# mryndzionek/composable-sdr

Measured on AMD Instinct MI355X. Metric: MS/s CF32 throughput, 256-ch PFB+FM pipeline, higher is better.
Workload: dtype f32; 1 GPU; cfg3: 256-ch firpfbch(m=7,As=80)+dcBlocker+freqdem(kf=0.3) on synthetic CF32, AGC off (-a 0), 262144 frames/step (512 MiB in, 256 MiB out), HBM-resident; channels=256, demod=fm, mix=False, route=fused-256|k_tile256<FM>, preheat_steps=11199, collective=none, rccl_ranks=1

## Files before the change

composable_sdr_amd/csrc/capi.hip:

```cpp
#include "../../include/csdr.h"
#include "csdr_internal.h"
#include "fused.h"

#include <cmath>
#include <cstdio>
#include <cstring>
#include <new>

namespace csdr {
const char *last_error();
}
using namespace csdr;

namespace {

struct DevGuard {
    int prev = -1; bool ok = true;
    DevGuard() = default;
    explicit DevGuard(int dev) { select(dev); }
    void select(int dev) {
        if (hipGetDevice(&prev) != hipSuccess) { ok = false; return; }
        if (dev >= 0 && dev != prev && hipSetDevice(dev) != hipSuccess) ok = false;
    }
    ~DevGuard() { if (prev >= 0) (void)hipSetDevice(prev); }
// ... 766 lines not shown
int csdr_symsync_get_taps(const csdr_symsync *h, float *mf, float *dmf)
{
    if (!h) return CSDR_ERR_INVALID;
    if (mf) std::memcpy(mf, h->d.mf.data(), sizeof(float) * h->d.mf.size());
    if (dmf) std::memcpy(dmf, h->d.dmf.data(), sizeof(float) * h->d.dmf.size());
    return CSDR_OK;
}

}

namespace {
constexpr uint32_t ST1 = 1u << 1, ST2 = 1u << 2, ST4 = 1u << 4, ST8 = 1u << 8, ST_ANY = ~0u;
struct RouteRow {
    uint32_t M;
    uint32_t strides;
    bool (*supported)(uint32_t M, uint32_t p);
    int (*create)(const FusedConfig &cfg, ChainPlan **out);
    const char *path_prefix;
    double dc_window;
    const char *name, *run_sized, *other, *agc_tail;
};
const RouteRow ROUTES[] = {
    {256, ST1 | ST2 | ST4 | ST8, plan256_supported, plan256_create, "fused-256|", 6 * 4096.0, "fused-256",
     "k_run256v2<FM | CF32[, G]> (whole band: calls of >= 1024 whole tiles of 16 frames; interleaved shards G = 2, 4, 8: every whole tile)",
     "k_tile256<FM | CF32> (look-back tile kernel: chunk-sized calls, ragged ends, and contiguous channel shards at every size) [+ k_shard_gather]",
     "channelizer -> CF32 plane (tile-major for run-sized calls of whole tiles) -> k_agc_spec_tm | k_agc_spec -> k_agc_fix [-> k_mix]"},
    {64, ST1, plan64_supported, plan64_create, "fused-", 6 * 4096.0, "fused-k_run64",
     "k_run64v2 (CF32 output, whole band, nf % 64 == 0, >= 8 tiles of 64 frames per run)", "k_run64<FM | CF32> (FM output, shards, ragged calls)",
     "k_run64v2 -> CF32 plane (tile-major, run-sized calls) -> k_agc_spec_tm | k_run64<CF32> -> k_agc_spec; -> k_agc_fix [-> k_mix]"},
    {1024, ST1 | ST2 | ST4 | ST8, plan1024_supported, plan1024_create, "fused-", 6 * 4096.0, "fused-k_run1024",
     "k_run1024v3<FM | CF32> (whole band, calls of whole 4-frame tiles; a call that ends inside a 128-byte line stores the front part of it); "
     "k_shard1024<FM | CF32, G> (interleaved shards G = 4, 8: fold of the aliasing branches behind the FIR + a (1024 / G)-point DFT across the lanes; run-sized calls of whole tiles); "
     "k_run1024v2<FM, 2> (interleaved shards G = 2, FM output)",
     "k_run1024<FM | CF32> (ragged calls, contiguous shards, the other calls of interleaved shards) [+ k_pfb1024_fixup, k_shard_gather1024]", "k_run1024v3<CF32> -> CF32 plane (tile-major) -> k_agc_spec_tm | k_run1024<CF32> -> k_agc_spec; -> k_agc_fix [-> k_mix]"},
    {4096, ST1, plan4096_supported, plan4096_create, "fused-4096|", 7 * 4096.0, "fused-4096",
     "k_front4096 (DC blocker + pre-mix + FIR, branch-tiled: four sibling workgroups per frame, radix-4 split of the DFT on the registers) -> z (8 B / sample) "
     "-> k_back4096<CF32 | FM | FM,mix> (four 1024-point DFTs per frame, 16-frame blocks, whole 128-byte lines per row) [-> k_mix4096_finish]; whole band; "
     "DeNo --mix without the AGC keeps the any-M route's mix identity",
     "the same kernels (any call size; short calls use fewer runs)", "k_front4096 -> k_back4096<CF32> -> CF32 plane (tile-major: calls of whole 16-frame blocks, >= 4096 frames) -> k_agc_spec_tm | k_agc_spec -> k_agc_fix [-> k_mix]"},
    {0, ST_ANY, nullptr, nullptr, nullptr, 0.0, "generic",
     "k_dc_tile -> k_pfb_fir (M = 1024, forced generic: k_pfb1024) -> k_fft_r16 | k_fft_pow2 | k_dft_direct [interleaved shard: k_fold + (M / G)-point DFT] "
     "-> k_transpose_fm | k_mix_frames | k_transpose;  DeNo --mix over all channels: k_dc_fold + k_mixid_finish (M % 4096 == 0) | k_dc_tile + k_branch0_fir "
     "(the sum of all bins of a frame is M x branch 0);  DeNo --mix of an interleaved shard (M % 4096 == 0, G = 2, 4, 8): k_dc_fold8 + k_mixid_shard_finish "
     "(the shard's channel sum is M / G x the phasor sum of the G surviving branches)",
     "the same kernels (any call size)", "... -> k_transpose -> k_agc_spec -> k_agc_fix [-> k_fm] [-> k_mix]"},
};
const RouteRow *route_select(uint32_t M, uint32_t p, uint32_t G, uint32_t flags, const DcParams *dc)
// ... 853 lines not shown
```

composable_sdr_amd/csrc/fused_common.h:

```cpp
#pragma once
#include "fused.h"

#include <cmath>
#include <cstdlib>
#include <vector>

namespace csdr {
namespace {

constexpr int M256 = 256;
constexpr int P = 14;
constexpr int NB = 16;
constexpr int FS_X = 272;
constexpr int FS_Z = 289;
constexpr int RS_Z = 18;
constexpr int RS_Y = 17;
constexpr int LDS_F2 = 16 * FS_Z;
constexpr int E_OFF = 4096;
constexpr int LOOKBACK = 10;
constexpr unsigned SPIN_LIMIT = 1u << 24;

typedef unsigned long long u64;
typedef float v2f __attribute__((ext_vector_type(2)));

// ... 330 lines not shown
__host__ __device__ __forceinline__ void run_range(const RunSplit &sp, uint32_t w, uint32_t &first, uint32_t &last)
{
    const uint32_t s = w / sp.rps, i = w - s * sp.rps;
    first = sp.base[s] + (uint32_t)((unsigned long long)i * sp.tiles[s] / sp.rps);
    last = sp.base[s] + (uint32_t)((unsigned long long)(i + 1) * sp.tiles[s] / sp.rps);
}

struct RunArgs {
    TileArgs t;
    RunSplit split;
    PhaseK pk;
    uint32_t nruns;
    float l2beta;
    uint32_t prio_div;
    uint32_t trace_light;
    const float4 *prev_tail;
    uint32_t indep;
    uint32_t pair_align;
    uint32_t wu_batch6;
    uint32_t wu, wu_rot;
    uint32_t tile_step;
    uint32_t nowu;
    float2 *cpre, *side;
};
constexpr int DCFIX_F = 113;

__device__ __forceinline__ float2 wg_sum(float2 v, float2 *red, int tid)
{
#pragma unroll
    for (int d = 32; d >= 1; d >>= 1) { v.x += __shfl_xor(v.x, d); v.y += __shfl_xor(v.y, d); }
    if ((tid & 63) == 0) red[tid >> 6] = v;
    __syncthreads();
    const float2 r = cadd(cadd(red[0], red[1]), cadd(red[2], red[3]));
    __syncthreads();
    return r;
}

__device__ __forceinline__ void row_scan4(float &x0, float &x1, float &x2, float &x3, float &s0, float &s1, float &s2, float &s3,
                                          float b1, float b2, float b4, float b8, float na)
{
    asm volatile(
        "v_mov_b32_e32 %4, %0\n\t"
        "v_mov_b32_e32 %5, %1\n\t"
        "v_mov_b32_e32 %6, %2\n\t"
        "v_mov_b32_e32 %7, %3\n\t"
        "v_fmac_f32_dpp %4, %4, %8 row_shr:1 row_mask:0xf bank_mask:0xf\n\t"
// ... 74 lines not shown
```

composable_sdr_amd/csrc/fused_v2_common.h:

```cpp
#pragma once
#include "fused_common.h"

namespace csdr {
namespace {

typedef float v4f __attribute__((ext_vector_type(4)));
#ifndef V2_DMA_AUX
#define V2_DMA_AUX ""
#endif
#ifndef V2_DMA_AUX_STREAM
#define V2_DMA_AUX_STREAM V2_DMA_AUX
#endif

__device__ __forceinline__ void bar()
{
    asm volatile("s_waitcnt lgkmcnt(0)\n\ts_barrier" ::: "memory");
}
__device__ __forceinline__ float opaque_v(float x) { asm volatile("" : "+v"(x)); return x; }

__device__ __forceinline__ unsigned dma_offset(int tid)
{
    const int wave = tid >> 6, lane = tid & 63;
    const int slot = 64 * wave + lane, q = slot >> 3, i = (slot & 7) ^ ((q >> 1) & 7);
    return (unsigned)(8 * q + i) * 16u;
// ... 90 lines not shown
    const v2f aA = mnA * rcA, aB = mnB * rcB;
    const v2f zA = aA * aA, zB = aB * aB;
    const v2f refv = {k.ref, k.ref};
    const v2f sA = aA * refv, sB = aB * refv;
    v2f pA = __builtin_elementwise_fma((v2f){k.c[7], k.c[7]}, zA, (v2f){k.c[6], k.c[6]});
    v2f pB = __builtin_elementwise_fma((v2f){k.c[7], k.c[7]}, zB, (v2f){k.c[6], k.c[6]});
#pragma unroll
    for (int i = 5; i >= 0; i--) {
        pA = __builtin_elementwise_fma(pA, zA, (v2f){k.c[i], k.c[i]});
        pB = __builtin_elementwise_fma(pB, zB, (v2f){k.c[i], k.c[i]});
    }
    const v2f tA = pA * sA, tB = pB * sB;
    const v2f hpv = {k.hp, k.hp}, piv = {k.pi, k.pi};
    const v2f thA = hpv - tA, thB = hpv - tB;
    const v2f uA = {sel_abs_gt(q[0].y, q[0].x, thA.x, tA.x), sel_abs_gt(q[1].y, q[1].x, thA.y, tA.y)};
    const v2f uB = {sel_abs_gt(q[2].y, q[2].x, thB.x, tB.x), sel_abs_gt(q[3].y, q[3].x, thB.y, tB.y)};
    const v2f wA = piv - uA, wB = piv - uB;
    m[0] = copysignf(sel_neg(q[0].x, wA.x, uA.x), q[0].y);
    m[1] = copysignf(sel_neg(q[1].x, wA.y, uA.y), q[1].y);
    m[2] = copysignf(sel_neg(q[2].x, wB.x, uB.x), q[2].y);
    m[3] = copysignf(sel_neg(q[3].x, wB.y, uB.y), q[3].y);
}

template <int CTRL> __device__ __forceinline__ float dpp_keep(float old, float v)
{
    return __int_as_float(__builtin_amdgcn_update_dpp(__float_as_int(old), __float_as_int(v), CTRL, 0xf, 0xf, false));
}

}
template <size_t OFF> __device__ __forceinline__ unsigned kernarg_u32_s()
{
    unsigned v = 0;
#if defined(__HIP_DEVICE_COMPILE__)
    typedef __attribute__((address_space(4))) const char *kptr;
    kptr ka = (kptr)__builtin_amdgcn_kernarg_segment_ptr();
    asm volatile("s_load_dword %0, %1, %2\n\ts_waitcnt lgkmcnt(0)" : "=s"(v) : "s"(ka), "n"(OFF) : "memory");
#endif
    return v;
}
template <size_t OFF> __device__ __forceinline__ float2 *kernarg_ptr_s()
{
    float2 *p = nullptr;
#if defined(__HIP_DEVICE_COMPILE__)
    typedef __attribute__((address_space(4))) const char *kptr;
    kptr ka = (kptr)__builtin_amdgcn_kernarg_segment_ptr();
    unsigned long long v;
// ... 8 lines not shown
```

composable_sdr_amd/csrc/kernels_fused.hip:

```cpp
#include "fused_common.h"
#include <cstring>

namespace csdr {

namespace {

#define STAMP(i) do { if (A.trace && tid == 0) A.trace[(size_t)b * 16 + (i)] = __builtin_amdgcn_s_memtime(); } while (0)

template <bool FM>
__global__ __launch_bounds__(256) void k_tile256(TileArgs A)
{
    __shared__ __attribute__((aligned(16))) float2 R[LDS_F2];
    __shared__ float2 tw_s[M256];
    __shared__ float2 Tt[2][16];
    __shared__ float2 carry_s[2];
    __shared__ unsigned tile_s;

    const int tid = threadIdx.x;
    if (tid == 0) tile_s = atomicAdd(A.ticket, 1u);
    tw_s[tid] = A.tw[tid];
    __syncthreads();
    const unsigned b = tile_s;
    if (b >= A.nb) return;
    STAMP(0);
// ... 267 lines not shown
{
    const unsigned i = blockIdx.x * 256u + threadIdx.x;
    dst[i] = src[i];
}

__global__ __launch_bounds__(64) void k_shard_gather(const float *__restrict__ src, float *__restrict__ dst, uint32_t c0, uint32_t G, uint32_t rem,
                                                     uint32_t nf, uint32_t t0, uint32_t w)
{
    const uint32_t m = blockIdx.x;
    for (uint32_t i = threadIdx.x; i < rem * w; i += 64) dst[((size_t)m * nf + t0) * w + i] = src[(size_t)(c0 + G * m) * rem * w + i];
}

struct FusedPlan : ChainPlan {
    using ChainPlan::ChainPlan;
    std::string kernel;
    uint32_t max_nb = 0, epoch = 0;
    float *d_taps = nullptr;
    float2 *d_tw = nullptr, *d_wpre = nullptr;
    float2 *d_yhist[2] = {nullptr, nullptr}, *d_vend[2] = {nullptr, nullptr}, *d_rp[2] = {nullptr, nullptr};
    unsigned *d_ticket = nullptr, *d_yflag = nullptr, *d_status = nullptr;
    u64 *d_agg = nullptr, *d_ylast = nullptr;
    float2 *d_cpre = nullptr, *d_side = nullptr, *d_rt = nullptr;
    bool nowu = false;
    u64 *d_trace = nullptr;
    uint32_t run_min_tiles = 1024;
    float slot_weight[8] = {1.f, 1.f, 1.f, 1.f, 1.f, 1.f, 1.f, 1.f};
    uint32_t resident_wgs_v2 = 512;
    bool use_v3 = false;
    float *d_shard_tail = nullptr;
    float4 *d_tail[3] = {nullptr, nullptr, nullptr};
    int tail_w = 0;
    bool tail_valid = false, save_tails = false;
    TileArgs proto;

    int init();
    const char *name() const override { return kernel.c_str(); }
    bool tile_major_ok(uint32_t nf) const override;
    void keep_tail() override { save_tails = cfg.G == 1; }
    bool can_overlap(uint32_t nf) const override;
    bool tail_recorded() const override { return save_tails && tail_valid; }
    int status(unsigned *st) override;
    int trace(unsigned long long *out, uint32_t ntiles) override;
    int reset_state(hipStream_t s) override;
    int run(const FusedCall &call, void *out, hipStream_t s, KernelTimer *timer) override;
    bool v2_call(uint32_t nf) const { return cfg.G == 1 && cfg.c0 == 0 && cfg.C == cfg.M && nf / NB >= run_min_tiles; }
};
// ... 79 lines not shown
    for (int i = 0; i < 3; i++) {
        if ((r = mem.alloc(&d_tail[i], sizeof(float4) * 2048 * (WU + 1)))) return r;
        CSDR_HIP(hipMemset(d_tail[i], 0, sizeof(float4) * 2048 * (WU + 1)));
    }
    tail_valid = true;
    if ((r = mem.alloc(&d_ticket, sizeof(unsigned)))) return r;
    if ((r = mem.alloc(&d_status, sizeof(unsigned)))) return r;
    if ((r = mem.alloc(&d_yflag, sizeof(unsigned) * max_nb))) return r;
    if ((r = mem.alloc(&d_agg, sizeof(u64) * 2 * max_nb))) return r;
    if ((r = mem.alloc(&d_ylast, sizeof(u64) * (size_t)cfg.M * max_nb))) return r;
    if (const char *e = diag_env("CSDR_RUN_MIN_TILES")) run_min_tiles = (uint32_t)atol(e);
    if (cfg.mix && (r = mem.alloc(&d_premix, (size_t)cfg.C * cfg.max_nf * (cfg.fm ? 4 : 8)))) return r;
    if (diag_env("CSDR_TRACE")) {
        if ((r = mem.alloc(&d_trace, sizeof(u64) * 16 * max_nb))) return r;
        CSDR_HIP(hipMemset(d_trace, 0, sizeof(u64) * 16 * max_nb));
    }
    nowu = cfg.G == 1 && cfg.c0 == 0 && cfg.C == cfg.M && cfg.dc_block && dc_window_ok(cfg.dc, (DCFIX_F - 1) * 256.0) &&
           !(diag_env("CSDR_NOWU") && atoi(diag_env("CSDR_NOWU")) == 0);
    if (nowu) {
        if ((r = mem.alloc(&d_cpre, sizeof(float2) * 2050))) return r;
        if ((r = mem.alloc(&d_side, sizeof(float2) * 2048 * 4 * DCFIX_F))) return r;
        if ((r = mem.alloc(&d_rt, sizeof(float2) * 2 * DCFIX_F * 4))) return r;
        CSDR_HIP(hipMemset(d_cpre, 0, sizeof(float2) * 2050));
    }
    CSDR_HIP(hipMemcpy(d_taps, cfg.taps, sizeof(float) * cfg.M * cfg.p, hipMemcpyHostToDevice));
    std::vector<float2> tw(cfg.M);
    for (uint32_t k1 = 0; k1 < 16; k1++)
        for (uint32_t b1 = 0; b1 < 16; b1++) {
            const double a = -2.0 * 3.14159265358979323846 * (double)(b1 * k1) / (double)cfg.M;
            tw[16 * k1 + b1] = make_float2((float)std::cos(a), (float)std::sin(a));
        }
    const std::vector<float2> wpre = premix_table();
    CSDR_HIP(hipMemcpy(d_tw, tw.data(), sizeof(float2) * cfg.M, hipMemcpyHostToDevice));
    CSDR_HIP(hipMemcpy(d_wpre, wpre.data(), sizeof(float2) * 2 * cfg.M, hipMemcpyHostToDevice));
    if (nowu) {
        std::vector<float2> rt((size_t)2 * DCFIX_F * 4);
        dc_state_response(cfg, wpre.data(), 15u, (uint32_t)DCFIX_F, 126u, rt.data());
        CSDR_HIP(hipMemcpy(d_rt, rt.data(), sizeof(float2) * rt.size(), hipMemcpyHostToDevice));
    }
    CSDR_HIP(hipMemset(d_status, 0, sizeof(unsigned)));
    CSDR_HIP(hipMemset(d_yflag, 0, sizeof(unsigned) * max_nb));
    CSDR_HIP(hipMemset(d_agg, 0, sizeof(u64) * 2 * max_nb));

    TileArgs &A = proto;
    A = TileArgs{};
    A.taps = d_taps; A.tw = d_tw; A.wpre = d_wpre;
// ... 71 lines not shown
        RA.t = A; RA.pk = phase_consts(c.fm_ref);
        uint32_t nruns = v3 ? cus : resident_wgs_v2;
        if (v3) { if (const char *e = diag_env("CSDR_V3_RUNS")) nruns = (uint32_t)atol(e); }
        if (nruns > A.nb / 8) nruns = A.nb / 8;
        if (nruns < 1) nruns = 1;
        RA.nruns = nruns;
        static const float v2_weight_cf[8] = {1.2f, 0.8f, 1.f, 1.f, 1.f, 1.f, 1.f, 1.f};
        static const float v2_weight_fm[8] = {1.24f, 0.76f, 1.f, 1.f, 1.f, 1.f, 1.f, 1.f};
        const float *v2_weight = c.fm ? v2_weight_fm : v2_weight_cf;
        static const float equal_weight[8] = {1.f, 1.f, 1.f, 1.f, 1.f, 1.f, 1.f, 1.f};
        static const bool pd_equal = diag_env("CSDR_PD_EQUAL") != nullptr;
        RA.split = make_split(A.nb, nruns, cus, (call.indep && pd_equal) ? equal_weight : ((v2 && !diag_env("CSDR_RUN_WEIGHTS")) ? v2_weight : slot_weight));
        { const char *e = diag_env("CSDR_PRIO_ROT"); RA.prio_div = e ? (atoi(e) ? cus : 0u) : (v2 ? 0u : cus); }
        { const char *e = diag_env("CSDR_TRACE"); RA.trace_light = (e && atoi(e) == 2) ? 1u : 0u; }
        { const char *e = diag_env("CSDR_WU"); RA.wu = e ? (uint32_t)atoi(e) : (uint32_t)WU; }
        { const char *e = diag_env("CSDR_WU_ROT"); RA.wu_rot = e ? (uint32_t)atoi(e) : 0u; }
        RA.pair_align = (v2 && (c.fm || diag_env("CSDR_PAIR_ALIGN_CF"))) ? 1u : 0u;
        { const char *e = diag_env("CSDR_WU_BATCH6"); RA.wu_batch6 = e ? (uint32_t)atoi(e) : 1u; }
        RA.l2beta = c.dc_block ? (float)std::log2((double)c.dc.beta) : -1000.0f;
        RA.tile_step = call.tile_major ? c.C * 128u : (uint32_t)NB * (c.fm ? 4u : 8u);
        const bool whole = nf == nb_full * NB;
        RA.indep = call.indep ? 1u : 0u;
        RA.nowu = (nowu && !shard && !v3 && !RA.indep && nruns >= 2 && nruns <= 2048) ? 1u : 0u;
        RA.cpre = d_cpre; RA.side = d_side;
        RA.prev_tail = d_tail[tail_w];
        if (save_tails && !shard && v2 && whole && nb_full >= WU + 1) {
            const int nxt = (tail_w + 1) % 3;
            static const bool nocopy = diag_env("CSDR_PD_NOCOPY") != nullptr;
            if (!nocopy) hipLaunchKernelGGL(k_save_tail, dim3(2048 * (WU + 1) / 256), dim3(256), 0, s,
                                            reinterpret_cast<const float4 *>(call.d_in + (size_t)(nb_full - (WU + 1)) * 4096), d_tail[nxt]);
            if (call.ev_tail) CSDR_HIP(hipEventRecord(call.ev_tail, s));
            tail_w = nxt; tail_valid = true;
        } else tail_valid = false;
        if (timer && (r = timer->begin(s))) return r;
        if (nb_full == 0) {  }
#ifdef CSDR_WITH_RUN256_V3
        else if (v3) { if ((r = run256_v3_launch(&RA, c.fm, nruns, s))) return r; }
#endif
        else if ((r = run256_v2_launch(&RA, c.fm, c.G, nruns, s))) return r;
        if (RA.nowu && nb_full && (r = run256_dcfix_launch(&RA, c.fm, nruns, d_rt, s))) return r;
        if (timer && (r = timer->end(s))) return r;
        const uint32_t rem = nf - nb_full * NB;
        if (rem) {
            if (nb_full) cur ^= 1;
            TileArgs T = proto;
            T.x = call.d_in + (size_t)nb_full * NB * c.M; T.out = A.out;
            if (shard) { T.c0 = 0; T.C = c.M; T.out = d_shard_tail; }
            T.yhist_in = d_yhist[cur]; T.yhist_out = d_yhist[cur ^ 1];
            T.vend_in = d_vend[cur];   T.vend_out = d_vend[cur ^ 1];
            T.rp_in = d_rp[cur];       T.rp_out = d_rp[cur ^ 1];
            if (++epoch == 0) epoch = 1;
            T.epoch = epoch; T.nf = rem; T.nb = 1; T.out_stride = nf; T.out_t0 = nb_full * NB;
            if (shard) { T.out_stride = rem; T.out_t0 = 0; }
            T.parity0 = (uint32_t)((frames_done + nb_full * NB) & 1);
            CSDR_HIP(hipMemsetAsync(d_ticket, 0, sizeof(unsigned), s));
            if (c.fm) hipLaunchKernelGGL(k_tile256<true>, dim3(1), dim3(256), 0, s, T);
            else hipLaunchKernelGGL(k_tile256<false>, dim3(1), dim3(256), 0, s, T);
            if (shard) hipLaunchKernelGGL(k_shard_gather, dim3(c.C), dim3(64), 0, s, (const float *)d_shard_tail, (float *)A.out, c.c0, c.G, rem,
                                          nf, nb_full * NB, c.fm ? 1u : 2u);
        }
    } else {
        kernel = c.fm ? "k_tile256<FM>" : "k_tile256<CF32>";
        tail_valid = false;
// ... 30 lines not shown
```

composable_sdr_amd/csrc/kernels_fused_v2.hip:

```cpp
#ifndef V2_FM_PACKED
#define V2_FM_PACKED 1
#endif
#ifndef V2_ABLATE
#define V2_ABLATE 0
#endif

#ifndef V2_COLSCAN
#define V2_COLSCAN 0
#endif
#ifndef V2_PAIR
#define V2_PAIR 1
#endif
#ifndef V2_STORE_AUX
#define V2_STORE_AUX ""
#endif
#ifndef V2_PAIR_CF
#define V2_PAIR_CF 0
#endif
#ifndef V2_BAR_E
#define V2_BAR_E 0
#endif
#ifndef V2_PAD
#define V2_PAD 1
#endif
// ... 3 lines not shown

#include "fused_v2_common.h"
#include <cstddef>
#include <type_traits>

namespace csdr {
namespace {

constexpr unsigned V2_FSB = 2048u + (V2_PAD ? 128u : 0u);
constexpr int V2_FS2 = (int)V2_FSB / 8;
constexpr int V2_BUF = 16 * V2_FS2;
constexpr int V2_STASH = 2 * V2_BUF;
constexpr int V2_F2 = V2_STASH + 256 + 32 + 256 + (V2_COLSCAN ? 512 : 0);
#define V2_ZSW(f) (V2_PAD ? (((f) >> 1) & 7) : ((f) & 7))
#ifndef V2_RSWN
#define V2_RSWN V2_PAD
#endif
#define V2_RSW(a) (V2_RSWN ? ((a) & 7) : (((a) >> 1) & 7))

struct V2Args {
    RunArgs r;
};

template <bool FM, int G>
__global__ __launch_bounds__(256, 2) void k_run256v2(V2Args VA)
{
    static_assert(G == 1 || G == 2 || G == 4 || G == 8, "interleaved shards: G = 2, 4, 8");
    constexpr int NK1 = 16 / G;
    const RunArgs &RA = VA.r;
    const TileArgs &A = RA.t;
    __shared__ __attribute__((aligned(16))) float2 L[V2_F2];
    float2 *R = L, *ST = L + V2_STASH, *Tt = ST + 256, *red = Tt + 16;
    float2 *tw_s = red + 16;
    float2 *TRc = tw_s + 256, *Ec = TRc + 256;
    (void)TRc; (void)Ec;
    float2 *H = L + V2_BUF;
    float2 *E = ST;
    const int tid = threadIdx.x, j = tid;
    const unsigned w = blockIdx.x;
    unsigned first, last;
    run_range(RA.split, w, first, last);
    if (RA.pair_align) {
        first &= ~1u;
        if (last != A.nb) last &= ~1u;
    }
    const float4 *x4 = reinterpret_cast<const float4 *>(A.x);
    const int col_off = 16 * (j >> 4) + 2 * (((j & 15) >> 1) ^ V2_RSW(j >> 4)) + (j & 1);
    const unsigned goff = V2_RSWN ? dma_offset_rsw(tid) : dma_offset(tid);
    const unsigned wave_u = (unsigned)__builtin_amdgcn_readfirstlane(tid >> 6);
    const unsigned lds_wave = (unsigned)(size_t)(__attribute__((address_space(3))) float2 *)R + V2_FSB * (wave_u >> 1) + 1024u * (wave_u & 1u);

#ifndef V2_TRACE
#define V2_TRACE 0
#endif
// ... 1 lines not shown
#define V2LSTAMP(i) do { if (A.trace && RA.trace_light && tid == 0) A.trace[(size_t)first * 16 + (i)] = __builtin_amdgcn_s_memrealtime(); } while (0)
#else
#define V2LSTAMP(i) do { } while (0)
#endif
    V2LSTAMP(0);
    const bool cold = w > 0 || RA.indep;
    const int halo = (int)first - 1;
    auto tile_ptr = [&](int t) -> const float4 * { return t >= 0 ? x4 + (size_t)t * 2048 : RA.prev_tail + (size_t)(WU + 1 + t) * 2048; };
    if (first < last) dma_tile<false, 2 * V2_FSB>(x4 + (size_t)first * 2048, goff, lds_wave);
    if (cold) dma_tile<false, 2 * V2_FSB>(tile_ptr(halo), goff, lds_wave + (unsigned)(V2_BUF * 8));
    float h[P];
#pragma unroll
    for (int n = 0; n < P; n++) h[n] = A.taps[(M256 - 1 - j) + n * M256];
    float2 Wa = A.wpre[(A.parity0 & 1) * M256 + j], Wb = A.wpre[((A.parity0 & 1) ^ 1) * M256 + j];
    if (G > 1) {
        const int n = ((j >> 4) * (int)A.c0) & 15;
        const float C1 = 0.92387953251128674f, S1 = 0.38268343236508977f, R2 = 0.70710678118654752f;
        const int m4 = n & 3, qd = n >> 2;
        const float2 e = m4 == 0 ? make_float2(1.f, 0.f) : (m4 == 1 ? make_float2(C1, -S1) : (m4 == 2 ? make_float2(R2, -R2) : make_float2(S1, -C1)));
        const float2 rot = qd == 0 ? e : (qd == 1 ? make_float2(e.y, -e.x) : (qd == 2 ? make_float2(-e.x, -e.y) : make_float2(-e.y, e.x)));
        Wa = cmul(Wa, rot); Wb = cmul(Wb, rot);
    }
    tw_s[tid] = A.tw[tid];
    float2 wa[NB], wb[NB];
#pragma unroll
    for (int f = 0; f < NB; f++) { wa[f] = make_float2(0.f, 0.f); wb[f] = make_float2(0.f, 0.f); }
    float2 c;
    float2 w2 = make_float2(0.f, 0.f);

    if (!cold) {
        c = A.vend_in[0];
#pragma unroll
        for (int f = 3; f < NB; f++) wa[f] = A.yhist_in[(f - 3) * M256 + j];
    } else {
        const int h0 = RA.nowu ? halo : (RA.indep ? halo - (int)RA.wu : (halo > (int)RA.wu ? halo - (int)RA.wu : 0));
        const unsigned nwu = (unsigned)(halo - h0);
        float4 raw[8];
        float wt0, wt1;
        {
            const int wave = tid >> 6, lane = tid & 63;
            const int slot = 64 * wave + lane, q = slot >> 3;
            const int i = (slot & 7) ^ ((q >> 1) & 7);
            const int n = 16 * q + 2 * i;
            wt0 = exp2f((float)(4095 - n) * RA.l2beta);
            wt1 = exp2f((float)(4094 - n) * RA.l2beta);
        }
// ... 72 lines not shown
            const float2 s2 = (n == P - 1) ? w2 : wa[NB - 1 - n];
            acc = __builtin_elementwise_fma((v2f){s2.x, s2.y}, (v2f){h[n], h[n]}, acc);
        }
        H[j] = to_f2(acc);
        __syncthreads();
        v2f vv[16];
        if (tid < 16) {
#pragma unroll
            for (int a = 0; a < 16; a++) vv[a] = to_v(H[16 * a + tid]);
            fft16_v(vv);
#pragma unroll
            for (int i = (G > 1 ? 0 : 1); i < 16; i++) vv[i] = cmul_v(vv[i], to_v(tw_s[16 * ((XIDX(i) + (G > 1 ? (int)A.c0 : 0)) & 15) + tid]));
#pragma unroll
            for (int i = 0; i < 16; i++) H[256 + 16 * XIDX(i) + tid] = to_f2(vv[i]);
        }
        __syncthreads();
        if (tid < 16) {
#pragma unroll
            for (int b = 0; b < 16; b++) vv[b] = to_v(H[256 + 16 * (G * (tid % NK1)) + b]);
            fft16_v(vv);
#pragma unroll
            for (int i = 0; i < 16; i++) ST[tid * 16 + i] = to_f2(vv[i]);
            if (G == 1 && RA.nowu) {
                if (tid >= 14) RA.side[((size_t)w * 4 + (tid - 14)) * DCFIX_F] = to_f2(vv[13]);
                else if (tid <= 1) RA.side[((size_t)w * 4 + 2 + tid) * DCFIX_F] = to_f2(vv[2]);
            }
        }
        __syncthreads();
    }

    const v2f Wav = to_v(Wa), Wbv = to_v(Wb);
    const float na = opaque_v(-A.alpha), be = opaque_v(A.beta);
    const float kJ = -A.alpha * exp2f((float)j * RA.l2beta);
    const float b256 = A.b256[1];
    const FmK2 fk = {{opaque_v(9.999993443e-01f), opaque_v(-3.332985938e-01f), opaque_v(1.994656026e-01f), opaque_v(-1.390860826e-01f),
                      opaque_v(9.642146528e-02f), opaque_v(-5.591168255e-02f), opaque_v(2.186254039e-02f), opaque_v(-4.054457881e-03f)},
                     opaque_v(1e-37f), opaque_v(A.fm_ref), opaque_v(RA.pk.hp), opaque_v(RA.pk.pi)};
    const int q = tid, sw = V2_RSW(q & 15);
    const unsigned raw_a = (unsigned)q * 128u + (unsigned)(q >> 4) * (V2_FSB - 2048u) + ((unsigned)sw << 4);
    const int f1 = tid >> 4, b1 = tid & 15;
    const int k1 = tid >> 4, f2 = tid & 15;
    const unsigned x_a = (unsigned)f1 * V2_FSB + (unsigned)b1 * 8u;
    const unsigned zw_a = (unsigned)f1 * V2_FSB + (unsigned)((((b1 >> 1) ^ V2_ZSW(f1)) << 1) | (b1 & 1)) * 8u;
    const unsigned z_a = (unsigned)f2 * V2_FSB + (unsigned)k1 * 128u + ((unsigned)V2_ZSW(f2) << 4);
    const int j1 = k1 % NK1, hb = (G == 8) ? ((k1 >> 1) & 1) : 0;
    const unsigned z_a_g = (unsigned)f2 * V2_FSB + (unsigned)(G * j1) * 128u + ((unsigned)V2_ZSW(f2) << 4);
    const uint32_t voff = ((uint32_t)(G == 1 ? k1 : j1 + 16 * hb) * A.out_stride + A.out_t0 + (uint32_t)f2) * (FM ? 4u : 8u);
    const size_t row16 = (size_t)NK1 * A.out_stride * (FM ? 4u : 8u);
#if V2_TRACE
#define V2STAMP(i) do { if (A.trace && !RA.trace_light && tid == 0) A.trace[(size_t)b_ * 16 + (i)] = __builtin_amdgcn_s_memtime(); } while (0)
#else
#define V2STAMP(i) do { } while (0)
#endif

    float hold[16];
    v2f holdc[V2_PAIR_CF ? 16 : 1];
    auto tile = [&](float2 (&old)[NB], float2 (&nw)[NB], unsigned b_, const int par) {
        unsigned b = (unsigned)__builtin_amdgcn_readfirstlane((int)b_);
        asm volatile("" : "+s"(b));
        char *B = reinterpret_cast<char *>(L) + par * (V2_BUF * 8);
        float2 *Bf = reinterpret_cast<float2 *>(B);
        if (RA.prio_div) {
            if (((b_ - first) + w / RA.prio_div) & 1u) __builtin_amdgcn_s_setprio(1); else __builtin_amdgcn_s_setprio(0);
        }
        V2STAMP(0);
        if (G == 1 && b + 1 == last && tid == 0) {
            if (kernarg_u32_s<offsetof(V2Args, r.nowu)>()) kernarg_ptr_s<offsetof(V2Args, r.cpre)>()[w + 1] = c;
        }
        if (V2_TRACE && A.trace && !RA.trace_light && tid == 0) A.trace[(size_t)b_ * 16 + 15] = __builtin_amdgcn_s_memrealtime();
        bar();
        V2STAMP(1);
#ifdef V2_SELECTIVE_POLICY
        if (!(V2_ABLATE & 1) && b + 1 < last) {
            if (b + 1 + (WU + 1) < last) dma_tile<true, 2 * V2_FSB>(x4 + (size_t)(b + 1) * 2048, goff, lds_wave + (unsigned)(par ^ 1) * (V2_BUF * 8u));
            else dma_tile<false, 2 * V2_FSB>(x4 + (size_t)(b + 1) * 2048, goff, lds_wave + (unsigned)(par ^ 1) * (V2_BUF * 8u));
        }
#else
        if (!(V2_ABLATE & 1) && b + 1 < last) dma_tile<false, 2 * V2_FSB>(x4 + (size_t)(b + 1) * 2048, goff, lds_wave + (unsigned)(par ^ 1) * (V2_BUF * 8u));
#endif
#if V2_COLSCAN
#pragma unroll
        for (int f = 0; f < NB; f++) nw[f] = Bf[V2_FS2 * f + col_off];
        col_run_scan(nw, TRc, A, tid);
        V2STAMP(2);
        bar();
        col_run_carries(TRc, Ec, Tt, A, tid);
        bar();
        V2STAMP(3);
        {
            v2f V = to_v(c);
            const float kj = -A.alpha * A.bj[j & 15];
            const v2f kJv = {kJ, kJ}, bv = {b256, b256}, kjv = {kj, kj};
#pragma unroll
            for (int f = 0; f < NB; f++) {
// ... 164 lines not shown
                    for (int u = 0; u < NS; u++) {
                        const char *rowp = obase + (size_t)XIDX(S0 + u) * row16;
                        asm volatile("s_nop 4\n\tglobal_store_dwordx2 %0, %1, %2\n\ts_nop 1" :: "v"(voff), "v"(y[u]), "s"(rowp) : "memory");
                    }
                }
            };
            if (G == 2) { if (wave_u < 2u) shard_tail(std::integral_constant<int, 0>{}); else shard_tail(std::integral_constant<int, 2>{}); }
            else switch (wave_u) {
                case 0: shard_tail(std::integral_constant<int, 0>{}); break;
                case 1: shard_tail(std::integral_constant<int, 1>{}); break;
                case 2: shard_tail(std::integral_constant<int, 2>{}); break;
                default: shard_tail(std::integral_constant<int, 3>{}); break;
            }
            V2STAMP(14);
            return;
        }
#pragma unroll
        for (int i = 0; i < 8; i++) {
            const v4f v = *reinterpret_cast<const v4f *>(B + (z_a ^ (unsigned)(i << 4)));
            vv[2 * i] = (v2f){v.x, v.y}; vv[2 * i + 1] = (v2f){v.z, v.w};
        }
        if (!(V2_ABLATE & 16)) fft16_v(vv);
        V2STAMP(11);
        if (G == 1 && cold && b - first < 7u && kernarg_u32_s<offsetof(V2Args, r.nowu)>()) {
            float2 *sd = kernarg_ptr_s<offsetof(V2Args, r.side)>() + ((size_t)w * 4) * DCFIX_F + 1 + 16 * (size_t)(b - first) + f2;
            if (k1 >= 14) sd[(k1 - 14) * DCFIX_F] = to_f2(vv[13]);
            else if (k1 <= 1) sd[(2 + k1) * DCFIX_F] = to_f2(vv[2]);
        }
        char *obase = reinterpret_cast<char *>(A.out) + (size_t)b * RA.tile_step;
        if (FM) {
            asm volatile("s_waitcnt vmcnt(0)" ::: "memory");
#pragma unroll
            for (int i = 0; i < 16; i += 4) {
                float2 rp[4], rr[4];
#pragma unroll
                for (int u = 0; u < 4; u += 2) {
                    const v4f sp = *reinterpret_cast<const v4f *>(ST + k1 * 16 + i + u);
                    rp[u] = make_float2(dpp_keep<0x111>(sp.x, vv[i + u].x), dpp_keep<0x111>(sp.y, vv[i + u].y));
                    rp[u + 1] = make_float2(dpp_keep<0x111>(sp.z, vv[i + u + 1].x), dpp_keep<0x111>(sp.w, vv[i + u + 1].y));
                    rr[u] = to_f2(vv[i + u]); rr[u + 1] = to_f2(vv[i + u + 1]);
                }
                float mq_[4];
                float (&mq)[4] = (V2_PAIR && par == 0) ? *reinterpret_cast<float (*)[4]>(&hold[i]) : mq_;
                if (V2_ABLATE & 4) { mq[0] = rp[0].x + rr[0].y; mq[1] = rp[1].y + rr[1].x; mq[2] = rp[2].x + rr[2].y; mq[3] = rp[3].y + rr[3].x; }
                else if (V2_FM_PACKED) fm_quad(rp, rr, fk, mq);
                else {
                    const FmK k1s = {fk.tiny, fk.ref, fk.hp, fk.pi};
#pragma unroll
                    for (int u = 0; u < 4; u++) mq[u] = fm_sample(rp[u], rr[u], k1s);
                }
                if (V2_PAIR && par == 0 && b + 1 < last) continue;
#pragma unroll
                for (int u = 0; u < 4; u++) {
                    const char *rowp = obase + (size_t)XIDX(i + u) * row16;
                    if (V2_ABLATE & 2) asm volatile("" :: "v"(mq[u]), "s"(rowp));
                    else {
                        if (V2_PAIR && par == 1) asm volatile(V2_SNOP "global_store_dword %0, %1, %2 offset:-64" V2_STORE_AUX :: "v"(voff), "v"(hold[i + u]), "s"(rowp) : "memory");
                        asm volatile(V2_SNOP "global_store_dword %0, %1, %2" V2_STORE_AUX :: "v"(voff), "v"(mq[u]), "s"(rowp) : "memory");
                    }
                }
            }
            if (f2 == 15) {
#pragma unroll
                for (int i = 0; i < 16; i += 2) *reinterpret_cast<v4f *>(ST + k1 * 16 + i) = (v4f){vv[i].x, vv[i].y, vv[i + 1].x, vv[i + 1].y};
            }
            V2STAMP(12);
            V2STAMP(13);
        } else {
            V2STAMP(12);
            asm volatile("s_waitcnt vmcnt(0)" ::: "memory");
            V2STAMP(13);
            if (V2_PAIR_CF && par == 0 && b + 1 < last) {
#pragma unroll
                for (int i = 0; i < 16; i++) holdc[i] = vv[i];
            } else {
#pragma unroll
                for (int i = 0; i < 16; i++) {
                    const char *rowp = obase + (size_t)XIDX(i) * row16;
                    if (V2_ABLATE & 2) asm volatile("" :: "v"(vv[i]), "s"(rowp));
                    else {
                        if (V2_PAIR_CF && par == 1) asm volatile(V2_SNOP "global_store_dwordx2 %0, %1, %2 offset:-128" V2_STORE_AUX :: "v"(voff), "v"(holdc[i]), "s"(rowp) : "memory");
                        asm volatile(V2_SNOP "global_store_dwordx2 %0, %1, %2" V2_STORE_AUX :: "v"(voff), "v"(vv[i]), "s"(rowp) : "memory");
                    }
                }
            }
        }
        V2STAMP(14);
    };

    V2LSTAMP(2);
    asm volatile("s_waitcnt vmcnt(0)" ::: "memory");
    V2LSTAMP(3);
    for (unsigned b = first; b < last; b += 2) {
        tile(wa, wb, b, 0);
        if (b + 1 >= last) break;
        tile(wb, wa, b + 1, 1);
    }

    V2LSTAMP(4);
    bar();
    if (FM) {
        const float2 lastY = ST[st_idx];
        if (last == A.nb && st_own) A.rp_out[tid] = lastY;
    }
    if (last == A.nb && tid == 0) A.vend_out[0] = c;
}

}

template <bool FM>
__global__ __launch_bounds__(128) void k_run256_dcfix(V2Args VA, const float2 *__restrict__ Rt)
{
    const RunArgs &RA = VA.r;
    const TileArgs &A = RA.t;
    __shared__ float2 Ys[4][DCFIX_F + 1];
    const unsigned w = blockIdx.x + 1;
    unsigned first, last;
    run_range(RA.split, w, first, last);
    if (RA.pair_align) { first &= ~1u; if (last != A.nb) last &= ~1u; }
    if (first >= last || first <= 1) return;
    const int t = threadIdx.x;
    const float2 c = RA.cpre[w];
    const float2 *R = Rt + (size_t)(A.parity0 & 1u) * DCFIX_F * 4;
    float2 y[4];
    if (t < DCFIX_F) {
#pragma unroll
        for (int ch = 0; ch < 4; ch++) {
            const float2 r = R[t * 4 + ch], s0 = RA.side[((size_t)w * 4 + ch) * DCFIX_F + t];
            y[ch] = make_float2(fmaf(c.x, r.x, fmaf(-c.y, r.y, s0.x)), fmaf(c.x, r.y, fmaf(c.y, r.x, s0.y)));
            Ys[ch][t] = y[ch];
        }
    }
    __syncthreads();
    if (t < 1 || t >= DCFIX_F) return;
    const unsigned b = first + (unsigned)(t - 1) / 16u, f2 = (unsigned)(t - 1) & 15u;
    if (b >= last) return;
    char *obase = reinterpret_cast<char *>(A.out) + (size_t)b * RA.tile_step;
    const FmK fk = {1e-37f, A.fm_ref, RA.pk.hp, RA.pk.pi};
#pragma unroll
    for (int ch = 0; ch < 4; ch++) {
        const size_t off = ((size_t)(126 + ch) * A.out_stride + A.out_t0 + f2) * (FM ? 4u : 8u);
        if (FM) *reinterpret_cast<float *>(obase + off) = fm_sample(Ys[ch][t - 1], y[ch], fk);
        else *reinterpret_cast<float2 *>(obase + off) = y[ch];
    }
}

int run256_dcfix_launch(const void *run_args, bool fm, unsigned nruns, const float2 *Rt, hipStream_t s)
{
    if (nruns < 2) return 0;
    V2Args VA;
    VA.r = *static_cast<const RunArgs *>(run_args);
    if (fm) hipLaunchKernelGGL(k_run256_dcfix<true>, dim3(nruns - 1), dim3(128), 0, s, VA, Rt);
    else hipLaunchKernelGGL(k_run256_dcfix<false>, dim3(nruns - 1), dim3(128), 0, s, VA, Rt);
    return 0;
}

static V2Args make_v2(const void *run_args)
{
    V2Args VA;
    VA.r = *static_cast<const RunArgs *>(run_args);
    return VA;
}

int run256_v2_launch(const void *run_args, bool fm, unsigned G, unsigned nruns, hipStream_t s)
{
    const V2Args VA = make_v2(run_args);
#define V2_LAUNCH(F, GG) hipLaunchKernelGGL((k_run256v2<F, GG>), dim3(nruns), dim3(256), 0, s, VA)
// ... 19 lines not shown
```

Baseline: 306,300 MS/s.

## Fold DC-correction fixup into run256v2 via inter-workgroup ready flags

```diff
diff --git a/composable_sdr_amd/csrc/capi.hip b/composable_sdr_amd/csrc/capi.hip
--- a/composable_sdr_amd/csrc/capi.hip
+++ b/composable_sdr_amd/csrc/capi.hip
@@ -812,7 +812,8 @@
 };
 const RouteRow ROUTES[] = {
     {256, ST1 | ST2 | ST4 | ST8, plan256_supported, plan256_create, "fused-256|", 6 * 4096.0, "fused-256",
-     "k_run256v2<FM | CF32[, G]> (whole band: calls of >= 1024 whole tiles of 16 frames; interleaved shards G = 2, 4, 8: every whole tile)",
+     "k_run256v2<FM | CF32[, G]> (whole band: calls of >= 1024 whole tiles of 16 frames, one launch: a run ends with the DC correction of its neighbour's "
+     "cold start; interleaved shards G = 2, 4, 8: every whole tile)",
      "k_tile256<FM | CF32> (look-back tile kernel: chunk-sized calls, ragged ends, and contiguous channel shards at every size) [+ k_shard_gather]",
      "channelizer -> CF32 plane (tile-major for run-sized calls of whole tiles) -> k_agc_spec_tm | k_agc_spec -> k_agc_fix [-> k_mix]"},
     {64, ST1, plan64_supported, plan64_create, "fused-", 6 * 4096.0, "fused-k_run64",
diff --git a/composable_sdr_amd/csrc/fused_common.h b/composable_sdr_amd/csrc/fused_common.h
--- a/composable_sdr_amd/csrc/fused_common.h
+++ b/composable_sdr_amd/csrc/fused_common.h
@@ -376,6 +376,9 @@
     uint32_t tile_step;
     uint32_t nowu;
     float2 *cpre, *side;
+    uint32_t *ready;
+    uint32_t epoch;
+    const float2 *rt;
 };
 constexpr int DCFIX_F = 113;
 
diff --git a/composable_sdr_amd/csrc/fused_v2_common.h b/composable_sdr_amd/csrc/fused_v2_common.h
--- a/composable_sdr_amd/csrc/fused_v2_common.h
+++ b/composable_sdr_amd/csrc/fused_v2_common.h
@@ -136,6 +136,55 @@
     m[3] = copysignf(sel_neg(q[3].x, wB.y, uB.y), q[3].y);
 }
 
+template <int N16> __device__ __forceinline__ void dma_small(const void *src, unsigned dst, int lane)
+{
+    asm volatile("" : "+s"(dst), "+v"(lane));
+    const unsigned loff = (unsigned)lane * 16u;
+#pragma unroll
+    for (int it = 0; it < (N16 + 63) / 64; it++) {
+        const unsigned d = dst + 1024u * (unsigned)it;
+        const char *sp = static_cast<const char *>(src) + 1024 * it;
+        unsigned keep;
+        if (64 * it + 64 <= N16 || lane < N16 - 64 * it)
+            asm volatile("s_mov_b32 %0, m0\n\ts_mov_b32 m0, %2\n\ts_nop 4\n\tglobal_load_lds_dwordx4 %1, %3\n\ts_mov_b32 m0, %0"
+                         : "=&s"(keep) : "v"(loff), "s"(d), "s"(sp) : "memory");
+    }
+}
+
+__device__ __forceinline__ void dma_word_wt(const unsigned *src, unsigned dst, int lane)
+{
+    asm volatile("" : "+s"(dst), "+v"(lane));
+    unsigned zero = 0u, keep;
+    if (lane == 0)
+        asm volatile("s_mov_b32 %0, m0\n\ts_mov_b32 m0, %2\n\ts_nop 4\n\tglobal_load_lds_dword %1, %3 sc1\n\ts_mov_b32 m0, %0"
+                     : "=&s"(keep) : "v"(zero), "s"(dst), "s"(src) : "memory");
+}
+
+__device__ __forceinline__ void store_wt(float2 *p, float2 v)
+{
+    __hip_atomic_store((__attribute__((address_space(1))) unsigned long long *)p, ((unsigned long long)__float_as_uint(v.y) << 32) | __float_as_uint(v.x),
+                       __ATOMIC_RELAXED, __HIP_MEMORY_SCOPE_AGENT);
+}
+__device__ __forceinline__ void publish_u32(unsigned *flag, unsigned v)
+{
+    __hip_atomic_store((__attribute__((address_space(1))) unsigned *)flag, v, __ATOMIC_RELAXED, __HIP_MEMORY_SCOPE_AGENT);
+}
+constexpr unsigned long long HANDOFF_WAIT_TICKS = 50000000ull;
+__device__ __forceinline__ bool wait_u32(const unsigned *flag, unsigned want)
+{
+    const unsigned long long t0 = __builtin_amdgcn_s_memrealtime();
+    for (;;) {
+        unsigned v;
+        const unsigned z = 0u;
+        asm volatile("global_load_dword %0, %1, %2 sc1\n\ts_waitcnt vmcnt(0)" : "=v"(v) : "v"(z), "s"(flag) : "memory");
+        if ((unsigned)__builtin_amdgcn_readfirstlane((int)v) == want) break;
+        if (__builtin_amdgcn_s_memrealtime() - t0 > HANDOFF_WAIT_TICKS) return false;
+        __builtin_amdgcn_s_sleep(16);
+    }
+    __builtin_amdgcn_fence(__ATOMIC_ACQUIRE, "agent");
+    return true;
+}
+
 template <int CTRL> __device__ __forceinline__ float dpp_keep(float old, float v)
 {
     return __int_as_float(__builtin_amdgcn_update_dpp(__float_as_int(old), __float_as_int(v), CTRL, 0xf, 0xf, false));
diff --git a/composable_sdr_amd/csrc/kernels_fused.hip b/composable_sdr_amd/csrc/kernels_fused.hip
--- a/composable_sdr_amd/csrc/kernels_fused.hip
+++ b/composable_sdr_amd/csrc/kernels_fused.hip
@@ -313,6 +313,8 @@
     u64 *d_agg = nullptr, *d_ylast = nullptr;
     float2 *d_cpre = nullptr, *d_side = nullptr, *d_rt = nullptr;
     bool nowu = false;
+    uint32_t *d_ready = nullptr;
+    bool dcfix_inline = true;
     u64 *d_trace = nullptr;
     uint32_t run_min_tiles = 1024;
     float slot_weight[8] = {1.f, 1.f, 1.f, 1.f, 1.f, 1.f, 1.f, 1.f};
@@ -438,6 +440,9 @@
         if ((r = mem.alloc(&d_side, sizeof(float2) * 2048 * 4 * DCFIX_F))) return r;
         if ((r = mem.alloc(&d_rt, sizeof(float2) * 2 * DCFIX_F * 4))) return r;
         CSDR_HIP(hipMemset(d_cpre, 0, sizeof(float2) * 2050));
+        if ((r = mem.alloc(&d_ready, sizeof(uint32_t) * 2052))) return r;
+        CSDR_HIP(hipMemset(d_ready, 0, sizeof(uint32_t) * 2052));
+        if (const char *e = diag_env("CSDR_DCFIX_INLINE")) dcfix_inline = atoi(e) != 0;
     }
     CSDR_HIP(hipMemcpy(d_taps, cfg.taps, sizeof(float) * cfg.M * cfg.p, hipMemcpyHostToDevice));
     std::vector<float2> tw(cfg.M);
@@ -555,7 +560,11 @@
         const bool whole = nf == nb_full * NB;
         RA.indep = call.indep ? 1u : 0u;
         RA.nowu = (nowu && !shard && !v3 && !RA.indep && nruns >= 2 && nruns <= 2048) ? 1u : 0u;
-        RA.cpre = d_cpre; RA.side = d_side;
+        RA.cpre = d_cpre; RA.side = d_side; RA.rt = d_rt;
+        if (RA.nowu && dcfix_inline && nb_full >= 8 * nruns) {
+            if (++epoch == 0) epoch = 1;
+            RA.ready = d_ready; RA.epoch = epoch;
+        } else if (RA.nowu) kernel += "+k_run256_dcfix";
         RA.prev_tail = d_tail[tail_w];
         if (save_tails && !shard && v2 && whole && nb_full >= WU + 1) {
             const int nxt = (tail_w + 1) % 3;
@@ -571,7 +580,7 @@
         else if (v3) { if ((r = run256_v3_launch(&RA, c.fm, nruns, s))) return r; }
 #endif
         else if ((r = run256_v2_launch(&RA, c.fm, c.G, nruns, s))) return r;
-        if (RA.nowu && nb_full && (r = run256_dcfix_launch(&RA, c.fm, nruns, d_rt, s))) return r;
+        if (RA.nowu && !RA.ready && nb_full && (r = run256_dcfix_launch(&RA, c.fm, nruns, d_rt, s))) return r;
         if (timer && (r = timer->end(s))) return r;
         const uint32_t rem = nf - nb_full * NB;
         if (rem) {
diff --git a/composable_sdr_amd/csrc/kernels_fused_v2.hip b/composable_sdr_amd/csrc/kernels_fused_v2.hip
--- a/composable_sdr_amd/csrc/kernels_fused_v2.hip
+++ b/composable_sdr_amd/csrc/kernels_fused_v2.hip
@@ -49,6 +49,31 @@
     RunArgs r;
 };
 
+template <bool FM, int NCH, class SideF, class RespF>
+__device__ __forceinline__ void dcfix_frames(const TileArgs &A, uint32_t tile_step, const FmK &fk, float2 c, int t, int ch0, unsigned first, unsigned last,
+                                             SideF side, RespF resp)
+{
+    if (t < 1 || t >= DCFIX_F) return;
+    const unsigned b = first + (unsigned)(t - 1) / 16u, f2 = (unsigned)(t - 1) & 15u;
+    if (b >= last) return;
+    char *obase = reinterpret_cast<char *>(A.out) + (size_t)b * tile_step;
+    auto corrected = [&](int tt, int ch) {
+        const float2 r = resp(tt, ch), s0 = side(ch, tt);
+        return make_float2(fmaf(c.x, r.x, fmaf(-c.y, r.y, s0.x)), fmaf(c.x, r.y, fmaf(c.y, r.x, s0.y)));
+    };
+#pragma unroll
+    for (int ch = 0; ch < NCH; ch++) {
+        const size_t off = ((size_t)(126 + ch0 + ch) * A.out_stride + A.out_t0 + f2) * (FM ? 4u : 8u);
+        const float2 y = corrected(t, ch0 + ch);
+        if (FM) *reinterpret_cast<float *>(obase + off) = fm_sample(corrected(t - 1, ch0 + ch), y, fk);
+        else *reinterpret_cast<float2 *>(obase + off) = y;
+    }
+}
+constexpr int FX_SIDE = 0, FX_RESP = 4 * DCFIX_F, FX_FLAG = 8 * DCFIX_F, FX_N = FX_FLAG + 2;
+constexpr int V2_FX = V2_F2;
+constexpr int DCFIX_N16 = 4 * DCFIX_F * 8 / 16;
+static_assert(4 * DCFIX_F * 8 % 16 == 0 && (V2_COLSCAN || 2 * (V2_FX + FX_N) * 8 <= 160 * 1024), "DC correction scratch");
+
 template <bool FM, int G>
 __global__ __launch_bounds__(256, 2) void k_run256v2(V2Args VA)
 {
@@ -56,7 +81,7 @@
     constexpr int NK1 = 16 / G;
     const RunArgs &RA = VA.r;
     const TileArgs &A = RA.t;
-    __shared__ __attribute__((aligned(16))) float2 L[V2_F2];
+    __shared__ __attribute__((aligned(16))) float2 L[V2_FX + FX_N];
     float2 *R = L, *ST = L + V2_STASH, *Tt = ST + 256, *red = Tt + 16;
     float2 *tw_s = red + 16;
     float2 *TRc = tw_s + 256, *Ec = TRc + 256;
@@ -104,6 +129,7 @@
         Wa = cmul(Wa, rot); Wb = cmul(Wb, rot);
     }
     tw_s[tid] = A.tw[tid];
+    if (G == 1 && tid == 0) L[V2_FX + FX_FLAG] = make_float2(0.f, 0.f);
     float2 wa[NB], wb[NB];
 #pragma unroll
     for (int f = 0; f < NB; f++) { wa[f] = make_float2(0.f, 0.f); wb[f] = make_float2(0.f, 0.f); }
@@ -222,8 +248,8 @@
 #pragma unroll
             for (int i = 0; i < 16; i++) ST[tid * 16 + i] = to_f2(vv[i]);
             if (G == 1 && RA.nowu) {
-                if (tid >= 14) RA.side[((size_t)w * 4 + (tid - 14)) * DCFIX_F] = to_f2(vv[13]);
-                else if (tid <= 1) RA.side[((size_t)w * 4 + 2 + tid) * DCFIX_F] = to_f2(vv[2]);
+                if (tid >= 14) store_wt(&RA.side[((size_t)w * 4 + (tid - 14)) * DCFIX_F], to_f2(vv[13]));
+                else if (tid <= 1) store_wt(&RA.side[((size_t)w * 4 + 2 + tid) * DCFIX_F], to_f2(vv[2]));
             }
         }
         __syncthreads();
@@ -238,6 +264,7 @@
                      opaque_v(1e-37f), opaque_v(A.fm_ref), opaque_v(RA.pk.hp), opaque_v(RA.pk.pi)};
     const int q = tid, sw = V2_RSW(q & 15);
     const unsigned raw_a = (unsigned)q * 128u + (unsigned)(q >> 4) * (V2_FSB - 2048u) + ((unsigned)sw << 4);
+    constexpr int V2_WAVE_OF_RAW = 64 * 128 + 4 * ((int)V2_FSB - 2048);
     const int f1 = tid >> 4, b1 = tid & 15;
     const int k1 = tid >> 4, f2 = tid & 15;
     const unsigned x_a = (unsigned)f1 * V2_FSB + (unsigned)b1 * 8u;
@@ -255,6 +282,29 @@
 
     float hold[16];
     v2f holdc[V2_PAIR_CF ? 16 : 1];
+    auto fix_due = [&]() -> bool {
+        unsigned w1 = w + 1, l_ = last;
+        asm volatile("" : "+s"(w1), "+s"(l_));
+        return kernarg_ptr_s<offsetof(V2Args, r.ready)>() != nullptr && w1 < kernarg_u32_s<offsetof(V2Args, r.nruns)>() && l_ > 1u;
+    };
+    auto fetch_fix = [&]() {
+        if (!fix_due()) return;
+        unsigned w1 = w + 1;
+        asm volatile("" : "+s"(w1));
+        float2 *F = L + V2_FX;
+        const unsigned epoch = kernarg_u32_s<offsetof(V2Args, r.epoch)>();
+        bool ok = true;
+        if ((unsigned)__builtin_amdgcn_readfirstlane(__float_as_int(F[FX_FLAG].x)) == epoch) __builtin_amdgcn_fence(__ATOMIC_ACQUIRE, "agent");
+        else ok = wait_u32(reinterpret_cast<unsigned *>(kernarg_ptr_s<offsetof(V2Args, r.ready)>()) + w1, epoch);
+        if (ok) {
+            const unsigned fx = (unsigned)(size_t)(__attribute__((address_space(3))) float2 *)F;
+            const float2 *sd = kernarg_ptr_s<offsetof(V2Args, r.side)>() + (size_t)w1 * 4 * DCFIX_F;
+            const float2 *rt = kernarg_ptr_s<offsetof(V2Args, r.rt)>() + (size_t)(kernarg_u32_s<offsetof(V2Args, r.t.parity0)>() & 1u) * 4 * DCFIX_F;
+            dma_small<DCFIX_N16>(sd, fx + FX_SIDE * 8u, tid);
+            dma_small<DCFIX_N16>(rt, fx + FX_RESP * 8u, tid);
+            if (tid == 0) F[FX_FLAG].y = 1.f;
+        } else if (tid == 0) atomicOr(reinterpret_cast<unsigned *>(kernarg_ptr_s<offsetof(V2Args, r.t.status)>()), 4u);
+    };
     auto tile = [&](float2 (&old)[NB], float2 (&nw)[NB], unsigned b_, const int par) {
         unsigned b = (unsigned)__builtin_amdgcn_readfirstlane((int)b_);
         asm volatile("" : "+s"(b));
@@ -270,6 +320,19 @@
         if (V2_TRACE && A.trace && !RA.trace_light && tid == 0) A.trace[(size_t)b_ * 16 + 15] = __builtin_amdgcn_s_memrealtime();
         bar();
         V2STAMP(1);
+        if (G == 1 && b + 3 == last && __builtin_amdgcn_readfirstlane((int)raw_a) == 0) {
+            if (fix_due()) dma_word_wt(reinterpret_cast<unsigned *>(kernarg_ptr_s<offsetof(V2Args, r.ready)>()) + w + 1,
+                                       (unsigned)(size_t)(__attribute__((address_space(3))) float2 *)(L + V2_FX + FX_FLAG), tid);
+        }
+        if (G == 1 && b + 1 == last) {
+            const float2 *F = L + V2_FX;
+            if (__builtin_amdgcn_readfirstlane(__float_as_int(F[FX_FLAG].y)) != 0) {
+                const FmK fk1 = {fk.tiny, fk.ref, fk.hp, fk.pi};
+                const float2 *S = F + FX_SIDE, *Rs = F + FX_RESP;
+                dcfix_frames<FM, 2>(A, RA.tile_step, fk1, c, 16 * (k1 & 7) + f2, 2 * (k1 >> 3), last, last + 7u,
+                                    [&](int ch, int t) { return S[ch * DCFIX_F + t]; }, [&](int t, int ch) { return Rs[t * 4 + ch]; });
+            }
+        }
 #ifdef V2_SELECTIVE_POLICY
         if (!(V2_ABLATE & 1) && b + 1 < last) {
             if (b + 1 + (WU + 1) < last) dma_tile<true, 2 * V2_FSB>(x4 + (size_t)(b + 1) * 2048, goff, lds_wave + (unsigned)(par ^ 1) * (V2_BUF * 8u));
@@ -480,14 +543,32 @@
         }
         if (!(V2_ABLATE & 16)) fft16_v(vv);
         V2STAMP(11);
-        if (G == 1 && cold && b - first < 7u && kernarg_u32_s<offsetof(V2Args, r.nowu)>()) {
-            float2 *sd = kernarg_ptr_s<offsetof(V2Args, r.side)>() + ((size_t)w * 4) * DCFIX_F + 1 + 16 * (size_t)(b - first) + f2;
-            if (k1 >= 14) sd[(k1 - 14) * DCFIX_F] = to_f2(vv[13]);
-            else if (k1 <= 1) sd[(2 + k1) * DCFIX_F] = to_f2(vv[2]);
-        }
+        unsigned drop = 0;
+        if (G == 1 && cold && b - first < 8u && kernarg_u32_s<offsetof(V2Args, r.nowu)>()) {
+            unsigned *rdy = reinterpret_cast<unsigned *>(kernarg_ptr_s<offsetof(V2Args, r.ready)>());
+            unsigned f_ = first;
+            asm volatile("" : "+s"(f_));
+            if (rdy && f_ > 1u) drop = (b - first < 7u ? 1u : 0u) | (((V2_PAIR && FM) || (V2_PAIR_CF && !FM)) && par == 1 ? 2u : 0u);
+            if (b - first < 7u) {
+                float2 *sd = kernarg_ptr_s<offsetof(V2Args, r.side)>() + ((size_t)w * 4) * DCFIX_F + 1 + 16 * (size_t)(b - first) + f2;
+                int k1o = k1;
+                asm volatile("" : "+v"(k1o));
+                if (k1o >= 14) store_wt(&sd[(k1o - 14) * DCFIX_F], to_f2(vv[13]));
+                else if (k1o <= 1) store_wt(&sd[(2 + k1o) * DCFIX_F], to_f2(vv[2]));
+                if (rdy && (b - first == 6u || b + 1 == last)) {
+                    asm volatile("s_waitcnt vmcnt(0)" ::: "memory");
+                    bar();
+                    if (tid == 0) publish_u32(rdy + w, kernarg_u32_s<offsetof(V2Args, r.epoch)>());
+                }
+            }
+        }
+        const int wraw = __builtin_amdgcn_readfirstlane((int)raw_a);
+        const unsigned dropw = (unsigned)__builtin_amdgcn_readfirstlane((int)(drop << (wraw == 3 * V2_WAVE_OF_RAW ? 0 : (wraw == 0 ? 2 : 4))));
+#define V2_MASKED(half, bit, st) "s_mov_b32 %0, " half "\n\ts_bitcmp1_b32 %4, " #bit "\n\ts_cselect_b32 " half ", 0, %0\n\t" st "\n\ts_mov_b32 " half ", %0"
         char *obase = reinterpret_cast<char *>(A.out) + (size_t)b * RA.tile_step;
         if (FM) {
             asm volatile("s_waitcnt vmcnt(0)" ::: "memory");
+            if (b + 3 == last && __builtin_amdgcn_readfirstlane((int)raw_a) == 0) fetch_fix();
 #pragma unroll
             for (int i = 0; i < 16; i += 4) {
                 float2 rp[4], rr[4];
@@ -513,6 +594,17 @@
                     const char *rowp = obase + (size_t)XIDX(i + u) * row16;
                     if (V2_ABLATE & 2) asm volatile("" :: "v"(mq[u]), "s"(rowp));
                     else {
+                        if (G == 1 && (i + u == 13 || i + u == 2)) {
+                            unsigned sv;
+                            if (i + u == 13) {
+                                if (V2_PAIR && par == 1) asm volatile(V2_MASKED("exec_hi", 1, "global_store_dword %1, %2, %3 offset:-64" V2_STORE_AUX) : "=&s"(sv) : "v"(voff), "v"(hold[i + u]), "s"(rowp), "s"(dropw) : "memory", "scc");
+                                asm volatile(V2_MASKED("exec_hi", 0, "global_store_dword %1, %2, %3" V2_STORE_AUX) : "=&s"(sv) : "v"(voff), "v"(mq[u]), "s"(rowp), "s"(dropw) : "memory", "scc");
+                            } else {
+                                if (V2_PAIR && par == 1) asm volatile(V2_MASKED("exec_lo", 3, "global_store_dword %1, %2, %3 offset:-64" V2_STORE_AUX) : "=&s"(sv) : "v"(voff), "v"(hold[i + u]), "s"(rowp), "s"(dropw) : "memory", "scc");
+                                asm volatile(V2_MASKED("exec_lo", 2, "global_store_dword %1, %2, %3" V2_STORE_AUX) : "=&s"(sv) : "v"(voff), "v"(mq[u]), "s"(rowp), "s"(dropw) : "memory", "scc");
+                            }
+                            continue;
+                        }
                         if (V2_PAIR && par == 1) asm volatile(V2_SNOP "global_store_dword %0, %1, %2 offset:-64" V2_STORE_AUX :: "v"(voff), "v"(hold[i + u]), "s"(rowp) : "memory");
                         asm volatile(V2_SNOP "global_store_dword %0, %1, %2" V2_STORE_AUX :: "v"(voff), "v"(mq[u]), "s"(rowp) : "memory");
                     }
@@ -527,6 +619,7 @@
         } else {
             V2STAMP(12);
             asm volatile("s_waitcnt vmcnt(0)" ::: "memory");
+            if (b + 3 == last && __builtin_amdgcn_readfirstlane((int)raw_a) == 0) fetch_fix();
             V2STAMP(13);
             if (V2_PAIR_CF && par == 0 && b + 1 < last) {
 #pragma unroll
@@ -537,6 +630,17 @@
                     const char *rowp = obase + (size_t)XIDX(i) * row16;
                     if (V2_ABLATE & 2) asm volatile("" :: "v"(vv[i]), "s"(rowp));
                     else {
+                        if (G == 1 && (i == 13 || i == 2)) {
+                            unsigned sv;
+                            if (i == 13) {
+                                if (V2_PAIR_CF && par == 1) asm volatile(V2_MASKED("exec_hi", 1, "global_store_dwordx2 %1, %2, %3 offset:-128" V2_STORE_AUX) : "=&s"(sv) : "v"(voff), "v"(holdc[i]), "s"(rowp), "s"(dropw) : "memory", "scc");
+                                asm volatile(V2_MASKED("exec_hi", 0, "global_store_dwordx2 %1, %2, %3" V2_STORE_AUX) : "=&s"(sv) : "v"(voff), "v"(vv[i]), "s"(rowp), "s"(dropw) : "memory", "scc");
+                            } else {
+                                if (V2_PAIR_CF && par == 1) asm volatile(V2_MASKED("exec_lo", 3, "global_store_dwordx2 %1, %2, %3 offset:-128" V2_STORE_AUX) : "=&s"(sv) : "v"(voff), "v"(holdc[i]), "s"(rowp), "s"(dropw) : "memory", "scc");
+                                asm volatile(V2_MASKED("exec_lo", 2, "global_store_dwordx2 %1, %2, %3" V2_STORE_AUX) : "=&s"(sv) : "v"(voff), "v"(vv[i]), "s"(rowp), "s"(dropw) : "memory", "scc");
+                            }
+                            continue;
+                        }
                         if (V2_PAIR_CF && par == 1) asm volatile(V2_SNOP "global_store_dwordx2 %0, %1, %2 offset:-128" V2_STORE_AUX :: "v"(voff), "v"(holdc[i]), "s"(rowp) : "memory");
                         asm volatile(V2_SNOP "global_store_dwordx2 %0, %1, %2" V2_STORE_AUX :: "v"(voff), "v"(vv[i]), "s"(rowp) : "memory");
                     }
@@ -558,8 +662,15 @@
     V2LSTAMP(4);
     bar();
     if (FM) {
-        const float2 lastY = ST[st_idx];
-        if (last == A.nb && st_own) A.rp_out[tid] = lastY;
+        if (G == 1) {
+            int tq = tid;
+            asm volatile("" : "+v"(tq));
+            const float2 lastY = ST[(tq & 15) * 16 + XIDX(tq >> 4)];
+            if (last == A.nb) A.rp_out[tq] = lastY;
+        } else {
+            const float2 lastY = ST[st_idx];
+            if (last == A.nb && st_own) A.rp_out[tid] = lastY;
+        }
     }
     if (last == A.nb && tid == 0) A.vend_out[0] = c;
 }
@@ -571,36 +682,16 @@
 {
     const RunArgs &RA = VA.r;
     const TileArgs &A = RA.t;
-    __shared__ float2 Ys[4][DCFIX_F + 1];
     const unsigned w = blockIdx.x + 1;
     unsigned first, last;
     run_range(RA.split, w, first, last);
     if (RA.pair_align) { first &= ~1u; if (last != A.nb) last &= ~1u; }
     if (first >= last || first <= 1) return;
-    const int t = threadIdx.x;
-    const float2 c = RA.cpre[w];
     const float2 *R = Rt + (size_t)(A.parity0 & 1u) * DCFIX_F * 4;
-    float2 y[4];
-    if (t < DCFIX_F) {
-#pragma unroll
-        for (int ch = 0; ch < 4; ch++) {
-            const float2 r = R[t * 4 + ch], s0 = RA.side[((size_t)w * 4 + ch) * DCFIX_F + t];
-            y[ch] = make_float2(fmaf(c.x, r.x, fmaf(-c.y, r.y, s0.x)), fmaf(c.x, r.y, fmaf(c.y, r.x, s0.y)));
-            Ys[ch][t] = y[ch];
-        }
-    }
-    __syncthreads();
-    if (t < 1 || t >= DCFIX_F) return;
-    const unsigned b = first + (unsigned)(t - 1) / 16u, f2 = (unsigned)(t - 1) & 15u;
-    if (b >= last) return;
-    char *obase = reinterpret_cast<char *>(A.out) + (size_t)b * RA.tile_step;
+    const float2 *S = RA.side + (size_t)w * 4 * DCFIX_F;
     const FmK fk = {1e-37f, A.fm_ref, RA.pk.hp, RA.pk.pi};
-#pragma unroll
-    for (int ch = 0; ch < 4; ch++) {
-        const size_t off = ((size_t)(126 + ch) * A.out_stride + A.out_t0 + f2) * (FM ? 4u : 8u);
-        if (FM) *reinterpret_cast<float *>(obase + off) = fm_sample(Ys[ch][t - 1], y[ch], fk);
-        else *reinterpret_cast<float2 *>(obase + off) = y[ch];
-    }
+    dcfix_frames<FM, 4>(A, RA.tile_step, fk, RA.cpre[w], (int)threadIdx.x, 0, first, last,
+                        [&](int ch, int t) { return S[ch * DCFIX_F + t]; }, [&](int t, int ch) { return R[t * 4 + ch]; });
 }
 
 int run256_dcfix_launch(const void *run_args, bool fm, unsigned nruns, const float2 *Rt, hipStream_t s)
```

Result: no change. 307,300 MS/s (median of 6 runs) (+0.3%).
